# creare-com/pydem

Hardware: AMD Instinct MI355X
Metric: Mcells/s (slope+aspect+UCA+TWI end-to-end) per tile; % HBM roofline (higher is better)
Workload: dtype f64

## Files before the change

pydem_amd/csrc/uca.hip:

```cpp
#include "uca_graph.h"
#include <algorithm>
#include <vector>
#include <math.h>
#include <stdlib.h>
#include <string.h>

#define PI_D 3.141592653589793

namespace {

__global__ __launch_bounds__(256) void k_section_proportion(const double *__restrict__ dir,
                                                            const uint8_t *__restrict__ flats,
                                                            const double *__restrict__ sec_theta, int64_t NN, int n, int m,
                                                            const double *__restrict__ elev,
                                                            int8_t *__restrict__ section, double *__restrict__ prop,
                                                            uint32_t *__restrict__ cinfo)
{
    (void)NN;
    for (int i = blockIdx.y; i < n; i += gridDim.y)
    for (int j = blockIdx.x * blockDim.x + threadIdx.x; j < m; j += gridDim.x * blockDim.x) {
        const int64_t c = (int64_t)i * m + j;
        const double theta = sec_theta[i];
        const double d = dir[c];
        int sec0 = (int)(int8_t)(int)floor(d / PI_D * 2.0);
// ... 431 lines not shown
    uint16_t list[TILE_RING];
    int tail;
    int limit;
};

__device__ __forceinline__ uint16_t &sp_of(TileW &L, int idx) { return reinterpret_cast<uint16_t *>(L.cs)[2 * idx]; }
__device__ __forceinline__ uint32_t sp_state(const TileW &L, int idx) { return (L.cs[idx] >> SP_STATE_SHIFT) & 3u; }

__device__ __forceinline__ uint32_t sp_dec(TileW &L, int idx) { return atomicSub(&L.cs[idx], 1u) & 0xFFFFu; }

__device__ __forceinline__ void tile_wave_sync()
{
    __builtin_amdgcn_fence(__ATOMIC_SEQ_CST, "workgroup");
    __builtin_amdgcn_wave_barrier();
}

__device__ __forceinline__ void tile_lds_sync()
{
    __builtin_amdgcn_fence(__ATOMIC_RELEASE, "workgroup", "local");
    __builtin_amdgcn_wave_barrier();
    __builtin_amdgcn_fence(__ATOMIC_ACQUIRE, "workgroup", "local");
}

constexpr int TILE_PEND = 48;
struct TileNext {
    int32_t *flag;
    int32_t *list, *count;
};

__device__ __forceinline__ const double *in_edge_ptr(const SweepArgs &A, int32_t c, int m, int d)
{
    const int q = d + (d >> 2);
    const int di = (q * 11) >> 5;
    const int32_t u = c + (di - 1) * m + (q - 3 * di - 1);
    return reinterpret_cast<const double *>(A.contrib + u) + (((0x5A >> d) & 1) ? 0 : 1);
}
__device__ __forceinline__ double in_edge(const SweepArgs &A, int32_t c, int m, int d) { return *in_edge_ptr(A, c, m, d); }

struct TileBase {
    const char *cinfo, *area, *contrib, *prop, *todo;
    int32_t org;
};
__device__ __forceinline__ TileBase tile_base(const SweepArgs &A, int i0, int j0)
{
    TileBase B;
    const int64_t org = (int64_t)(i0 - 1) * A.m + (j0 - 1);
// ... 69 lines not shown
            L.fin[HH - 1] = ((br >> 32) << 1) | ((bk >> 2) & 1ull) | (((bk >> 3) & 1ull) << 33);
        }
    }
    constexpr int STG_B = PYDEM_STG_B;
#pragma unroll 1
    for (int kb = 0; kb < NSET; kb += STG_B) {
        uint32_t wst[STG_B];
#pragma unroll
        for (int k = 0; k < STG_B; k++) wst[k] = stage_word(i0 + 2 * (kb + k) + half, j0 + l32);
#pragma unroll
        for (int k = 0; k < STG_B; k++) {
            const int r = 2 * (kb + k);
            const bool f = final_before(wst[k]);
            L.cs[lane + 64 * (kb + k)] = ((wst[k] == 0xFFFFFFFFu ? 0u : (wst[k] & CI_STATIC_MASK)) << 16) | ((f ? 1u : 0u) << SP_STATE_SHIFT);
            const unsigned long long b = __ballot(f);
            if (lane == 0) {
                L.fin[r + 1] = ((b & 0xFFFFFFFFull) << 1) | ((colL >> r) & 1ull) | (((colR >> r) & 1ull) << 33);
                L.fin[r + 2] = ((b >> 32) << 1) | ((colL >> (r + 1)) & 1ull) | (((colR >> (r + 1)) & 1ull) << 33);
            }
        }
    }
}

template <bool LISTED, bool WT = false>
__device__ __forceinline__ void sweep_one_tile(const SweepArgs &A, TileW &L, uint32_t pass, int tiles_x, int tid, int lane,
                                               uint8_t *__restrict__ tile_done, int32_t &n_final, const TileNext &N,
                                               int32_t *pend, int &npend, const int32_t *nbr16)
{
    const int by = tid / tiles_x, bx = tid - by * tiles_x;
    const int i0 = by * TH, j0 = bx * TT, n = A.n, m = A.m;
    const TileBase B = tile_base(A, i0, j0);
    const int half = lane >> 5, l32 = lane & 31;
    auto push_ready = [&](int cell, int consumed) {
        const int slot = atomicAdd(&L.tail, 1);
        if (slot - consumed < TILE_RING) L.list[slot % TILE_RING] = (uint16_t)cell;
        else atomicMin(&L.limit, slot);
    };
#ifdef PYDEM_TILE_PROF
    const bool prof = (A.dbg & 4) != 0 && (int)pass >= (A.dbg >> 8);
#else
    constexpr bool prof = false;
#endif
    long long tk0 = 0, tk1 = 0, tk2 = 0, tk3 = 0;
    int nrounds = 0;
    if (prof) tk0 = wall_clock64();
    if (lane == 0) { L.tail = 0; L.limit = INT32_MAX; }
    const double a0_row = (!WT && lane < TH && i0 + lane < n) ? A.a0[i0 + lane] : 0.0;
    constexpr int NSET = TH * TT / 64;
    tile_stage(A, B, L, pass, i0, j0, lane);
    tile_wave_sync();
    if (prof) tk1 = wall_clock64();
    uint32_t pitmask = 0;
    int32_t n_open = 0;
#pragma unroll 2
    for (int k = 0; k < NSET; k++) {
        const int li = 2 * k + half + 1, idx = lane + 64 * k;
        const uint32_t w = L.cs[idx];
        if (!((w >> SP_STATE_SHIFT) & 3u)) {
            const unsigned long long f0 = L.fin[li - 1], f1 = L.fin[li], f2 = L.fin[li + 1];
            const uint32_t nf = ((uint32_t)(f0 >> l32) & 7u) | (((uint32_t)(f1 >> l32) & 1u) << 3) |
                                (((uint32_t)(f1 >> (l32 + 2)) & 1u) << 4) | (((uint32_t)(f2 >> l32) & 7u) << 5);
            const uint32_t pend = __popc((w >> 16) & 0xFFu & ~nf);
            sp_of(L, idx) = (uint16_t)pend;
            n_open++;
            if (w & (CI_PIT_IN << 16)) pitmask |= 1u << k;
            else if (pend == 0) push_ready(lane + 64 * k, 0);
        }
    }
    if (pitmask) {
        constexpr int PB = 4;
#pragma unroll 1
        for (int kb = 0; kb < NSET; kb += PB) {
            if (!((pitmask >> kb) & ((1u << PB) - 1u))) continue;
            int32_t e0[PB];
#pragma unroll
            for (int k = 0; k < PB; k++) {
                e0[k] = 0;
                if (pitmask & (1u << (kb + k))) {
                    const int cell = lane + 64 * (kb + k);
                    e0[k] = ld_off<int2>(B.area, halo_cell((cell >> 5) + 1, (cell & 31) + 1, m) * 8u).x;
                }
            }
#pragma unroll
            for (int k = 0; k < PB; k++) {
                if (!(pitmask & (1u << (kb + k)))) continue;
                const int cell = lane + 64 * (kb + k);
                const int32_t c = B.org + (int32_t)halo_cell((cell >> 5) + 1, (cell & 31) + 1, m);
                const int idx = cell;
                uint32_t pend = sp_of(L, idx);
// ... 26 lines not shown
    int32_t finalized = 0;
    uint32_t wake = 0;
    int head = 0;
    int mycell = -1, cd = -1;
    double cv = 0.0;
    for (;;) {
        const int tail = L.tail < L.limit ? L.tail : L.limit;
        const bool need = mycell < 0;
        const unsigned long long nb = __ballot(need);
        const int rank = __builtin_amdgcn_mbcnt_hi((uint32_t)(nb >> 32), __builtin_amdgcn_mbcnt_lo((uint32_t)nb, 0u));
        const int avail = tail - head, wanted = __popcll(nb);
        if (need && rank < avail) { mycell = L.list[(head + rank) % TILE_RING]; cd = -1; }
        head += wanted < avail ? wanted : avail;
        if (!__ballot(mycell >= 0)) break;
        nrounds++;
        int next = -1, nd = -1;
        double nv = 0.0;
        if (mycell >= 0) {
            const int cell = mycell;
            const int li = (cell >> 5) + 1, lj = (cell & 31) + 1, idx = cell;
            const int gi = i0 + li - 1, gj = j0 + lj - 1;
            const uint32_t h = halo_cell(li, lj, m);
            const int32_t c = B.org + (int32_t)h;
            const uint32_t cw = L.cs[idx] >> 16;
            double pv = 0.0;
            if (cw & (CI_OUT1 | CI_OUT2)) pv = ld_off<double>(B.prop, h * 8u);
            int2 po = make_int2(0, 0);
            if (cw & (CI_PIT_IN | CI_PIT_OUT)) po = ld_off<int2>(B.area, h * 8u);
            uint32_t mm = cw & 0xFFu;
            double xs[4];
#pragma unroll
            for (int q = 0; q < 4; q++) {
                xs[q] = 0.0;
                if (mm) {
                    const int d = __ffs(mm) - 1; mm &= mm - 1u;
                    if (d == cd) xs[q] = cv; else xs[q] = in_edge_h(B, nbr16, h, d);
                }
            }
            double a;
            bool td;
            if constexpr (WT) {
                a = A.a0[c];
                td = false;
#pragma unroll
                for (int q = 0; q < 4; q++) a += xs[q];
            } else {
                a = L.a0[li - 1];
                td = (gi == 0 || gi == n - 1 || gj == 0 || gj == m - 1) && ld_off<uint8_t>(B.todo, h) != 0;
#pragma unroll
                for (int q = 0; q < 4; q++) { a += fabs(xs[q]); td = td || (xs[q] < 0); }
            }
            while (mm) {
                const int d = __ffs(mm) - 1; mm &= mm - 1u;
                const double x = (d == cd) ? cv : in_edge_h(B, nbr16, h, d);
                if constexpr (WT) a += x;
                else { a += fabs(x); td = td || (x < 0); }
            }
            if (cw & CI_PIT_IN)
                for (int32_t e = po.x; e < A.n_pit && A.pin_dst[e] == c; e++) {
                    const int32_t sc = A.pin_src[e];
                    a += A.area[sc] * A.pin_w[e];
                    if constexpr (!WT) td = td || (A.todo_work[sc] != 0);
                }
            double2 o = make_double2(0.0, 0.0);
            if (cw & CI_OUT1) o.x = a * pv;
            if (cw & CI_OUT2) o.y = a * (1 - pv);
            if (td) { o.x = -o.x; o.y = -o.y; }
            st_off<double>(B.area, h * 8u, a);
#ifndef PYDEM_EXP_NOCONTRIB
            st_off<double2>(B.contrib, h * 16u, o);
#endif
            if (LISTED) st_off<uint32_t>(B.cinfo, h * 4u, ci_with_level(cw, pass));
            if (td) st_off<uint8_t>(B.todo, h, (uint8_t)1);
            sp_of(L, idx) = (uint16_t)(2u << SP_STATE_SHIFT);
            finalized++;
            auto release = [&](int ti, int tj, double share, bool chainable) {
                if (ti >= 1 && ti <= TH && tj >= 1 && tj <= TT) {
                    const int tcell = (ti - 1) * TT + (tj - 1);
                    if (sp_dec(L, tcell) == 1u) {
                        if (chainable && next < 0) {
                            const int q = (li - ti + 1) * 3 + (lj - tj + 1);
                            next = tcell; nd = q - (q > 4 ? 1 : 0); nv = share;
                        } else push_ready(tcell, head);
                    }
                } else if (LISTED) {
                    const int dti = ti < 1 ? -1 : (ti > TH ? 1 : 0), dtj = tj < 1 ? -1 : (tj > TT ? 1 : 0);
                    if (ti >= 1 - TH && ti <= 2 * TH && tj >= 1 - TT && tj <= 2 * TT) wake |= 1u << ((dti + 1) * 3 + dtj + 1);
                    else {
                        const int tt = ((i0 + ti - 1) / TH) * tiles_x + (j0 + tj - 1) / TT;
                        if (atomicExch(&N.flag[tt], (int32_t)pass + 1) != (int32_t)pass + 1) N.list[atomicAdd(N.count, 1)] = tt;
                    }
                }
            };
            const int sct = ci_section(cw);
            if (cw & CI_OUT1) release(li + fe1r(sct), lj + fe1c(sct), o.x, true);
            if (cw & CI_OUT2) release(li + fe2r(sct), lj + fe2c(sct), o.y, true);
            if (cw & CI_PIT_OUT)
                for (int32_t e = po.y; e < A.n_pit && A.pit_src[e] == c; e++) {
                    const int32_t dc = A.pit_dst[e];
                    const int ti = dc / m - i0 + 1, tj = dc % m - j0 + 1;
                    release(ti, tj, 0.0, false);
                }
        }
        mycell = next; cd = nd; cv = nv;
        tile_wave_sync();
    }
    if (prof) tk3 = wall_clock64();
    if (!LISTED)
        for (int k = 0; k < NSET; k++) {
            const int li = 2 * k + half + 1, idx = lane + 64 * k;
            const uint32_t w = L.cs[idx];
            if (((w >> SP_STATE_SHIFT) & 3u) == 2u) A.cinfo[(int64_t)(i0 + li - 1) * m + j0 + l32] = ci_with_level(w >> 16, pass);
        }
    for (int off = 32; off > 0; off >>= 1) { finalized += __shfl_down(finalized, off); n_open += __shfl_down(n_open, off); }
    if (LISTED) {
        for (int off = 32; off > 0; off >>= 1) wake |= __shfl_xor(wake, off);
        bool win = false;
        int tt = 0;
        if (lane < 9 && ((wake >> lane) & 1u)) { tt = tid + (lane / 3 - 1) * tiles_x + (lane % 3 - 1); win = true; }
        if (lane == 9 && L.limit != INT32_MAX) { tt = tid; win = true; }
        if (win) win = atomicExch(&N.flag[tt], (int32_t)pass + 1) != (int32_t)pass + 1;
        const unsigned long long bw = __ballot(win);
        if (win) pend[npend + __popcll(bw & ((1ull << lane) - 1ull))] = tt;
        npend += __popcll(bw);
    }
    if (lane == 0) {
        n_final += finalized;
        if (finalized == n_open) tile_done[tid] = 1;
        A.tile_open[tid] = n_open - finalized;
        if (prof) {
            const long long tk4 = wall_clock64();
            unsigned long long *acc = reinterpret_cast<unsigned long long *>(A.err + (CS_TILE_PROF - CS_QUEUE_ERR));
            atomicAdd(acc + 0, (unsigned long long)(tk1 - tk0)); atomicAdd(acc + 1, (unsigned long long)(tk2 - tk1));
            atomicAdd(acc + 2, (unsigned long long)(tk3 - tk2)); atomicAdd(acc + 3, (unsigned long long)(tk4 - tk3));
            atomicAdd(acc + 4, (unsigned long long)nrounds); atomicAdd(acc + 5, 1ull);
            if (finalized == 0) atomicAdd(acc + 6, 1ull);
        }
    }
    tile_wave_sync();
}

#include "uca_sym.inl"

#ifndef PYDEM_SWEEP_STEAL
#define PYDEM_SWEEP_STEAL 1
#endif
#ifndef PYDEM_FULL_WPB
#define PYDEM_FULL_WPB 4
#endif
constexpr int FWPB = PYDEM_FULL_WPB;
template <bool LISTED, bool WT = false>
__global__ __launch_bounds__(64 * FWPB, 32 / FWPB) void k_sweep_tiles(SweepArgs A, uint32_t pass, int tiles_x, int tiles_total,
                                                     uint8_t *__restrict__ tile_done, int32_t *n_final, TileNext N, int32_t *work8)
{
    __shared__ TileW L[FWPB];
    __shared__ int32_t s_pend[FWPB][TILE_PEND];
    __shared__ int32_t s_nbr16[8];
    fill_nbr16(s_nbr16, A.m);
    __syncthreads();
    const int wave = __builtin_amdgcn_readfirstlane(threadIdx.x >> 6), lane = threadIdx.x & 63;
    int32_t fin = 0;
    int npend = 0;
    auto flush = [&]() {
        tile_wave_sync();
        int32_t base = 0;
// ... 23 lines not shown
            if (tile_done[tid]) continue;
            sweep_one_tile<LISTED, WT>(A, L[wave], pass, tiles_x, tid, lane, tile_done, fin, N, s_pend[wave], npend, s_nbr16);
            if (LISTED && npend > TILE_PEND - 10) flush();
        }
    }
#endif
    if (LISTED && npend) flush();
    if (lane == 0 && fin) atomicAdd(n_final, fin);
}

#ifndef PYDEM_LISTED_OCC
#define PYDEM_LISTED_OCC 6
#endif
#ifndef PYDEM_LISTED_WPB
#define PYDEM_LISTED_WPB 2
#endif
constexpr int LWPB = PYDEM_LISTED_WPB;
template <bool WT = false>
__global__ __launch_bounds__(64 * LWPB, PYDEM_LISTED_OCC) void k_sweep_tiles_listed(SweepArgs A, uint32_t pass, int tiles_x, const int32_t *__restrict__ list_in,
                                                            const int32_t *n_in, uint8_t *__restrict__ tile_done, int32_t *n_final,
                                                            TileNext N, int32_t *clear_count, int32_t *work3, SymArgs Y)
{
    __shared__ TileW L[LWPB];
    __shared__ SymLight SL[LWPB];
    const int wave = threadIdx.x >> 6, lane = threadIdx.x & 63;
    const int32_t nt = *n_in;
#ifdef PYDEM_LISTED_DYNAMIC
    if (blockIdx.x == 0 && threadIdx.x < 8) work3[((pass + 1) % 3) * 8 + threadIdx.x] = 0;
#endif
    if (blockIdx.x == 0 && threadIdx.x == 0) *clear_count = 0;
    __shared__ int32_t s_pend[LWPB][TILE_PEND];
    __shared__ int32_t s_nbr16[8];
    fill_nbr16(s_nbr16, A.m);
    __syncthreads();
    int32_t fin = 0;
    int npend = 0;
    auto flush = [&]() {
        tile_wave_sync();
        int32_t base = 0;
        if (lane == 0) base = atomicAdd(N.count, npend);
        base = __shfl(base, 0);
        if (lane < npend) N.list[base + lane] = s_pend[wave][lane];
        npend = 0;
        tile_wave_sync();
    };
#ifndef PYDEM_LISTED_DYNAMIC
    (void)work3;
    for (int32_t k = __builtin_amdgcn_readfirstlane(blockIdx.x * LWPB + wave); k < nt; k += gridDim.x * LWPB) {
#else
    const int xcd = blockIdx.x & 7;
    const int32_t per = (nt + 7) >> 3;
    int32_t *wk = &work3[(pass % 3) * 8 + xcd];
    for (;;) {
        int32_t k = 0;
        if (lane == 0) k = atomicAdd(wk, 1);
        k = __builtin_amdgcn_readfirstlane(__shfl(k, 0));
        (void)per;
        k = k * 8 + xcd;
        if (k >= nt) break;
#endif
        const int tid = __builtin_amdgcn_readfirstlane(list_in[k]);
        const uint32_t blk = Y.tile_sym ? __builtin_amdgcn_readfirstlane(Y.tile_sym[tid]) : SYM_NONE;
        if (blk != SYM_NONE) sym_light_visit<WT>(A, Y, SL[wave], pass, tiles_x, tid, lane, blk, fin, N, s_pend[wave], npend);
        else sweep_one_tile<true, WT>(A, L[wave], pass, tiles_x, tid, lane, tile_done, fin, N, s_pend[wave], npend, s_nbr16);
        if (npend > TILE_PEND - 10) flush();
    }
    if (npend) flush();
    if (lane == 0 && fin) atomicAdd(n_final, fin);
}

constexpr int DENSE_BAND = 64;
__global__ __launch_bounds__(256) void k_sweep_dense_level(SweepArgs A, uint32_t p, int32_t *n_final)
{
    const int n = A.n, m = A.m;
    int32_t fin = 0;
    const int j = blockIdx.x * blockDim.x + threadIdx.x;
    const int i_end = min(n, (int)(blockIdx.y + 1) * DENSE_BAND);
    if (j < m)
    for (int i = blockIdx.y * DENSE_BAND; i < i_end; i++) {
        const int32_t c = i * m + j;
        const uint32_t w = A.cinfo[c];
        const uint32_t lv = ci_level(w);
        if (lv >= 1 && lv != CI_LEVEL_INF) continue;
        const uint32_t cw = w & CI_STATIC_MASK;
        bool ready = true;
#pragma unroll
        for (int d = 0; d < 8; d++)
// ... 47 lines not shown
constexpr int RCAP = 256;
constexpr uint32_t RS_TAINT = 1u << 19, RS_FIN = 1u << 20;
constexpr int RS_OPEN_SHIFT = 11, RS_FINAL_SHIFT = 21;
constexpr uint32_t RS_CELL = (1u << RS_OPEN_SHIFT) - 1u, RS_CELL_OPEN = (1u << 19) - 1u;

struct TileR {
    TileW W;
    uint16_t map[TH * TT];
    double Kd[RCAP];
    double Pd[RCAP];
    uint32_t sm[RCAP];
};

__device__ __forceinline__ int nb_local(int cell, int d)
{
    const int q = d + (d >> 2);
    const int di = (q * 11) >> 5;
    return cell + (di - 1) * TT + (q - 3 * di - 1);
}

template <bool WT = false>
__device__ __forceinline__ void sweep_tile_resident(const SweepArgs &A, TileR &R, uint32_t pass, int tiles_x, int tid, int lane,
                                                    uint8_t *__restrict__ tile_done, int32_t &n_final, const TileNext &N,
                                                    int32_t *pend, int &npend)
{
    TileW &L = R.W;
    const int by = tid / tiles_x, bx = tid - by * tiles_x;
    const int i0 = by * TH, j0 = bx * TT, n = A.n, m = A.m;
    const int half = lane >> 5, l32 = lane & 31;
    constexpr int NSET = TH * TT / 64;
    if (lane == 0) L.tail = 0;
    const double a0_row = (!WT && lane < TH && i0 + lane < n) ? A.a0[i0 + lane] : 0.0;
    tile_stage(A, tile_base(A, i0, j0), L, pass, i0, j0, lane);
    tile_wave_sync();
    uint32_t pitmask = 0;
    int nslot = 0;
#pragma unroll 2
    for (int k = 0; k < NSET; k++) {
        const int li = 2 * k + half + 1, idx = lane + 64 * k;
        const uint32_t w = L.cs[idx];
        const bool open = !((w >> SP_STATE_SHIFT) & 3u);
        const unsigned long long bo = __ballot(open);
        if (open) {
            const unsigned long long f0 = L.fin[li - 1], f1 = L.fin[li], f2 = L.fin[li + 1];
            const uint32_t nf = ((uint32_t)(f0 >> l32) & 7u) | (((uint32_t)(f1 >> l32) & 1u) << 3) |
                                (((uint32_t)(f1 >> (l32 + 2)) & 1u) << 4) | (((uint32_t)(f2 >> l32) & 7u) << 5);
            const uint32_t im = (w >> 16) & 0xFFu;
            const uint32_t cnt = __popc(im & ~nf);
            sp_of(L, idx) = (uint16_t)cnt;
            const int s = nslot + __popcll(bo & ((1ull << lane) - 1ull));
            R.map[idx] = (uint16_t)s;
            R.sm[s] = (uint32_t)idx | ((im & ~nf) << RS_OPEN_SHIFT) | ((im & nf) << RS_FINAL_SHIFT);
            if (w & (CI_PIT_IN << 16)) pitmask |= 1u << k;
            else if (cnt == 0) L.list[atomicAdd(&L.tail, 1)] = (uint16_t)s;
        }
        nslot += __popcll(bo);
    }
    if (pitmask) {
#pragma unroll 1
        for (int k = 0; k < NSET; k++) {
            if (!(pitmask & (1u << k))) continue;
            const int cell = lane + 64 * k;
            const int32_t c = (i0 + (cell >> 5)) * m + j0 + (cell & 31);
            uint32_t cnt = sp_of(L, cell);
            for (int32_t e = pit_stash(A, c).x; e < A.n_pit && A.pin_dst[e] == c; e++) {
                const int32_t sc = A.pin_src[e];
                const int si = sc / m - i0, sj = sc % m - j0;
                if (si >= 0 && si < TH && sj >= 0 && sj < TT) cnt += sp_state(L, si * TT + sj) ? 0u : 1u;
                else { const uint32_t lv = ci_level(A.cinfo[sc]); if (!(lv >= 1 && lv < pass)) cnt |= SP_BLOCKED; }
            }
            sp_of(L, cell) = (uint16_t)cnt;
            if (cnt == 0) L.list[atomicAdd(&L.tail, 1)] = R.map[cell];
        }
    }
    tile_wave_sync();
    if (lane < TH) L.a0[lane] = a0_row;
    tile_wave_sync();
    for (int s = lane; s < nslot; s += 64) {
        uint32_t smv = R.sm[s];
        const int cell = smv & RS_CELL;
        const int gi = i0 + (cell >> 5), gj = j0 + (cell & 31);
        const int32_t c = gi * m + gj;
        const uint32_t cw = L.cs[cell] >> 16;
        double pv = 0.0;
        if (cw & (CI_OUT1 | CI_OUT2)) pv = A.prop[c];
        bool td = !WT && (gi == 0 || gi == n - 1 || gj == 0 || gj == m - 1) && A.todo_work[c] != 0;
        uint32_t mm = (smv >> RS_FINAL_SHIFT) & 0xFFu;
        double xs[4];
#pragma unroll
        for (int q = 0; q < 4; q++) {
            xs[q] = 0.0;
            if (mm) { const int d = __ffs(mm) - 1; mm &= mm - 1u; xs[q] = in_edge(A, c, m, d); }
        }
        double K;
        if constexpr (WT) {
// ... 1 lines not shown
#pragma unroll
            for (int q = 0; q < 4; q++) K += xs[q];
            while (mm) { const int d = __ffs(mm) - 1; mm &= mm - 1u; K += in_edge(A, c, m, d); }
        } else {
            K = L.a0[cell >> 5];
#pragma unroll
            for (int q = 0; q < 4; q++) { K += fabs(xs[q]); td = td || (xs[q] < 0); }
            while (mm) { const int d = __ffs(mm) - 1; mm &= mm - 1u; const double x = in_edge(A, c, m, d); K += fabs(x); td = td || (x < 0); }
        }
        R.Kd[s] = K; R.Pd[s] = pv;
        R.sm[s] = (smv & RS_CELL_OPEN) | (td ? RS_TAINT : 0u);
    }
    tile_lds_sync();
    uint32_t wake = 0;
    int head = 0;
    for (;;) {
        const int tail = L.tail;
        if (head >= tail) break;
        const int idx = head + lane;
        if (idx < tail) {
            const int s = L.list[idx];
            const uint32_t smv = R.sm[s];
            const int cell = smv & RS_CELL, li = cell >> 5, lj = cell & 31;
            const uint32_t cw = L.cs[cell] >> 16;
            double a = R.Kd[s];
            bool td = (smv & RS_TAINT) != 0u;
            uint32_t mm = (smv >> RS_OPEN_SHIFT) & 0xFFu;
            while (mm) {
                const int d = __ffs(mm) - 1; mm &= mm - 1u;
                const int ss = R.map[nb_local(cell, d)];
                const double as = R.Kd[ss], ps = R.Pd[ss];
                a += ((0x5A >> d) & 1) ? as * ps : as * (1 - ps);
                td = td || (R.sm[ss] & RS_TAINT);
            }
            const int32_t c = (i0 + li) * m + j0 + lj;
            int2 po = make_int2(0, 0);
            if (cw & (CI_PIT_IN | CI_PIT_OUT)) po = pit_stash(A, c);
            if (cw & CI_PIT_IN)
                for (int32_t e = po.x; e < A.n_pit && A.pin_dst[e] == c; e++) {
                    const int32_t sc = A.pin_src[e];
                    const int si = sc / m - i0, sj = sc % m - j0;
                    bool here = false;
                    if (si >= 0 && si < TH && sj >= 0 && sj < TT) here = sp_state(L, si * TT + sj) == 2u;
                    if (here) { const int ss = R.map[si * TT + sj]; a += R.Kd[ss] * A.pin_w[e]; td = td || (R.sm[ss] & RS_TAINT); }
                    else { a += A.area[sc] * A.pin_w[e]; if constexpr (!WT) td = td || (A.todo_work[sc] != 0); }
                }
            R.Kd[s] = a;
            R.sm[s] = (smv & RS_CELL) | (td ? RS_TAINT : 0u) | RS_FIN;
            sp_of(L, cell) = (uint16_t)(2u << SP_STATE_SHIFT);
            auto release = [&](int ti, int tj) {
                if (ti >= 0 && ti < TH && tj >= 0 && tj < TT) {
                    const int tcell = ti * TT + tj;
                    if (sp_dec(L, tcell) == 1u) L.list[atomicAdd(&L.tail, 1)] = R.map[tcell];
                } else {
                    const int dti = ti < 0 ? -1 : (ti >= TH ? 1 : 0), dtj = tj < 0 ? -1 : (tj >= TT ? 1 : 0);
                    if (ti >= -TH && ti < 2 * TH && tj >= -TT && tj < 2 * TT) wake |= 1u << ((dti + 1) * 3 + dtj + 1);
                    else {
                        const int tt = ((i0 + ti) / TH) * tiles_x + (j0 + tj) / TT;
                        if (atomicExch(&N.flag[tt], (int32_t)pass + 1) != (int32_t)pass + 1) N.list[atomicAdd(N.count, 1)] = tt;
                    }
                }
            };
            const int sct = ci_section(cw);
            if (cw & CI_OUT1) release(li + fe1r(sct), lj + fe1c(sct));
            if (cw & CI_OUT2) release(li + fe2r(sct), lj + fe2c(sct));
            if (cw & CI_PIT_OUT)
                for (int32_t e = po.y; e < A.n_pit && A.pit_src[e] == c; e++) {
                    const int32_t dc = A.pit_dst[e];
                    release(dc / m - i0, dc % m - j0);
                }
        }
        head = tail < head + 64 ? tail : head + 64;
        tile_lds_sync();
    }
    int nfin = 0;
    for (int s = lane; s < nslot; s += 64) {
        const uint32_t smv = R.sm[s];
        if (!(smv & RS_FIN)) continue;
        const int cell = smv & RS_CELL;
        const int32_t c = (i0 + (cell >> 5)) * m + j0 + (cell & 31);
        const uint32_t cw = L.cs[cell] >> 16;
        const double a = R.Kd[s], pv = R.Pd[s];
        double2 o = make_double2(0.0, 0.0);
        if (cw & CI_OUT1) o.x = a * pv;
        if (cw & CI_OUT2) o.y = a * (1 - pv);
        if (smv & RS_TAINT) { o.x = -o.x; o.y = -o.y; A.todo_work[c] = 1; }
        A.area[c] = a;
        A.contrib[c] = o;
        A.cinfo[c] = ci_with_level(cw, pass);
        nfin++;
    }
    for (int off = 32; off > 0; off >>= 1) { nfin += __shfl_down(nfin, off); wake |= __shfl_xor(wake, off); }
    bool win = false;
    int tt = 0;
    if (lane < 9 && ((wake >> lane) & 1u)) { tt = tid + (lane / 3 - 1) * tiles_x + (lane % 3 - 1); win = true; }
    if (win) win = atomicExch(&N.flag[tt], (int32_t)pass + 1) != (int32_t)pass + 1;
    const unsigned long long bw = __ballot(win);
    if (win) pend[npend + __popcll(bw & ((1ull << lane) - 1ull))] = tt;
    npend += __popcll(bw);
    if (lane == 0) {
        n_final += nfin;
        A.tile_open[tid] = nslot - nfin;
        if (nfin == nslot) tile_done[tid] = 1;
    }
    tile_wave_sync();
}

template <bool WT = false>
__global__ __launch_bounds__(64) void k_sweep_tiles_resident(SweepArgs A, uint32_t pass, int tiles_x, const int32_t *__restrict__ list_in,
                                                             const int32_t *n_in, uint8_t *__restrict__ tile_done, int32_t *n_final,
                                                             TileNext N, int32_t *clear_count, SymArgs Y)
{
    __shared__ TileR R;
    __shared__ SymLight SL;
    __shared__ int32_t s_pend[TILE_PEND];
    __shared__ int32_t s_nbr16[8];
    fill_nbr16(s_nbr16, A.m);
    __syncthreads();
    const int lane = threadIdx.x;
    const int32_t nt = *n_in;
    if (blockIdx.x == 0 && lane == 0) *clear_count = 0;
    int32_t fin = 0;
    int npend = 0;
    auto flush = [&]() {
        tile_wave_sync();
        int32_t base = 0;
        if (lane == 0) base = atomicAdd(N.count, npend);
        base = __shfl(base, 0);
        if (lane < npend) N.list[base + lane] = s_pend[lane];
        npend = 0;
        tile_wave_sync();
    };
    for (int32_t k = blockIdx.x; k < nt; k += gridDim.x) {
        const int tid = __builtin_amdgcn_readfirstlane(list_in[k]);
        const uint32_t blk = Y.tile_sym ? __builtin_amdgcn_readfirstlane(Y.tile_sym[tid]) : SYM_NONE;
        if (blk != SYM_NONE) sym_light_visit<WT>(A, Y, SL, pass, tiles_x, tid, lane, blk, fin, N, s_pend, npend);
        else if (__builtin_amdgcn_readfirstlane(A.tile_open[tid]) <= RCAP)
            sweep_tile_resident<WT>(A, R, pass, tiles_x, tid, lane, tile_done, fin, N, s_pend, npend);
        else
            sweep_one_tile<true, WT>(A, R.W, pass, tiles_x, tid, lane, tile_done, fin, N, s_pend, npend, s_nbr16);
        if (npend > TILE_PEND - 10) flush();
    }
    if (npend) flush();
    if (lane == 0 && fin) atomicAdd(n_final, fin);
}

constexpr uint32_t FC_COUNT = 0xFu, FC_BLOCKED = 1u << 8, FC_DONE = 1u << 9, FC_TODO = 1u << 10;

struct TileFirst {
    double2 slot[TT * TT];
    uint32_t cs[TT * TT];
    double a0[TT];
};

__device__ __forceinline__ void lds_sync()
{
    __builtin_amdgcn_fence(__ATOMIC_RELEASE, "workgroup", "local");
    __builtin_amdgcn_s_barrier();
    __builtin_amdgcn_fence(__ATOMIC_ACQUIRE, "workgroup", "local");
}

__global__ __launch_bounds__(256) void k_sweep_first(SweepArgs A, int tiles_x, int tiles_total, uint8_t *__restrict__ tile_done,
                                                     int32_t *n_final)
// ... 960 lines not shown
```

pydem_amd/csrc/uca_graph.h:

```cpp
#pragma once
#include "internal.h"
#include <stdlib.h>

namespace {

constexpr uint32_t CI_OUT1 = 1u << 8, CI_OUT2 = 1u << 9, CI_PIT_OUT = 1u << 10, CI_PIT_IN = 1u << 11;
constexpr int CI_SEC_SHIFT = 12, CI_LEVEL_SHIFT = 15;
constexpr uint32_t CI_LEVEL_INF = 0x1FFFFu, CI_STATIC_MASK = 0x7FFFu;
__device__ __forceinline__ uint32_t ci_level(uint32_t w) { return w >> CI_LEVEL_SHIFT; }
__device__ __forceinline__ int ci_section(uint32_t w) { return (int)((w >> CI_SEC_SHIFT) & 7u); }
__device__ __forceinline__ uint32_t ci_with_level(uint32_t w, uint32_t lv) { return (w & CI_STATIC_MASK) | (lv << CI_LEVEL_SHIFT); }

__device__ __constant__ const int NB_DI[8] = {-1, -1, -1, 0, 0, 1, 1, 1};
__device__ __constant__ const int NB_DJ[8] = {-1, 0, 1, -1, 1, -1, 0, 1};
__device__ __constant__ const int NB_S0[8] = {6, 5, 4, 0, 3, 0, 1, 2};
__device__ __constant__ const int NB_S1[8] = {7, 6, 5, 7, 4, 1, 2, 3};

__device__ __forceinline__ bool keep_edge(double w, double z_to, double z_from)
{
    return !isnan(w) && (w > 1e-8) && (z_to <= z_from);
}

struct SweepArgs {
    uint32_t *cinfo;
    const double *prop, *a0;
    double *area;
    double2 *contrib;
    uint8_t *todo_work;
    int n, m;
    const int32_t *pit_src, *pit_dst;
    const int32_t *pin_dst, *pin_src; const double *pin_w;
    int64_t n_pit;
    int dbg;
    int32_t qcap;
    int32_t *err;
    int32_t *tile_open;
};

struct QE { int32_t c; uint32_t cw; };

enum CounterSlot : int {
    CS_FRONTIER = 0,
    CS_PROCESSED = 3,
    CS_SOURCES = 4,
    CS_ROUNDS = 5,
    CS_EDGE_REACHED = 6,
    CS_EDGE_CLEARED = 7,
    CS_EDGE_SEEDS = 8,
    CS_CASCADE_STATE = 12,
    CS_SWEEP_STATE = 14,
    CS_QUEUE_ERR = 15,
    CS_WINDOW = 16,
    CS_H_CB_TOTALS = 16,
    CS_WORK = 16, CS_WORK_WORDS = 24,
    CS_TILE_PROF = 32, CS_TILE_PROF_WORDS = 24,
    CS_EINC_PROF = 40,
// ... 9 lines not shown
static_assert(CS_FRONTIER + 3 <= CS_PROCESSED && CS_ROUNDS == CS_PROCESSED + 2, "kernels reach the round count through the processed-cells pointer");
static_assert(CS_ROUNDS < CS_EDGE_REACHED && CS_EDGE_SEEDS < CS_CASCADE_STATE && CS_CASCADE_STATE < CS_SWEEP_STATE && CS_SWEEP_STATE < CS_QUEUE_ERR,
              "the scalars of a cascade are live together");
static_assert(CS_QUEUE_ERR < CS_WINDOW && CS_WINDOW <= CS_WORK, "one copy of the window shows the host every scalar of a cascade, and no scratch");
static_assert(CS_WORK + CS_WORK_WORDS <= CS_EINC_PROF, "zeroing the per-tile scratch leaves the fix-up's words alone");
static_assert(CS_TILE_PROF + CS_TILE_PROF_WORDS <= CS_TILE_LIST, "the visit profile ends before the tile lists");
static_assert(CS_EINC_PROF + 8 <= CS_ND_COUNT && CS_ND_COUNT + 2 <= CS_ND_NEXT && CS_ND_NEXT < CS_NAN_SEEDS && CS_NAN_SEEDS < CS_COND_EDGES
              && CS_COND_EDGES < CS_TILE_LIST, "the fix-up's words are live together and stay clear of the sweep's");
static_assert(CS_TILE_LIST + 4 <= CS_RESEED && CS_RESEED + 3 <= CS_END && CS_FLAT_SAVE + 2 <= CS_END, "the sweep's lists and replay words are live together");

inline int grid_for(int64_t work, int cap) { const int64_t g = cdiv(work, 256); return (int)(g < cap ? (g > 0 ? g : 1) : cap); }
}

static void fill_sweep_args(pydem_tile *t, SweepArgs &A)
{
    A.cinfo = t->cinfo; A.prop = t->prop; A.a0 = t->row_area; A.area = t->uca;
    A.contrib = (double2 *)t->contrib; A.todo_work = t->todo_work; A.n = (int)t->n; A.m = (int)t->m;
    A.pit_src = t->pits.src; A.pit_dst = t->pits.dst; A.n_pit = t->pits.n_edges;
    A.pin_dst = t->pits.in_dst; A.pin_src = t->pits.in_src; A.pin_w = t->pits.in_w;
    A.qcap = (int32_t)(t->NN / 2 < INT32_MAX ? t->NN / 2 : INT32_MAX);
    A.err = t->counters + CS_QUEUE_ERR;
    A.tile_open = nullptr;
    { const char *e = getenv("PYDEM_TILE_DEBUG"); A.dbg = e ? atoi(e) : 0; }
}
```

Before: 5750.

## Stage pit edge lists in LDS during listed tile sweeps

```diff
diff --git a/pydem_amd/csrc/uca.hip b/pydem_amd/csrc/uca.hip
--- a/pydem_amd/csrc/uca.hip
+++ b/pydem_amd/csrc/uca.hip
@@ -477,6 +477,69 @@
     __builtin_amdgcn_fence(__ATOMIC_ACQUIRE, "workgroup", "local");
 }
 
+constexpr int PS_CAP = 120;
+constexpr int PS_CELLS = 64;
+constexpr int PS_END = 0xFF;
+constexpr uint32_t CW_STAGED = 1u << 15;
+constexpr int SP_HEAD_SHIFT = 6;
+constexpr uint32_t SP_STAGED_COUNT = (1u << SP_HEAD_SHIFT) - 1u, SP_STAGED_READY = (3u << SP_STATE_SHIFT) | SP_BLOCKED | SP_STAGED_COUNT;
+constexpr int32_t PS_NBR = TH * TT, PS_FAR = 1 << 30;
+static_assert((CI_STATIC_MASK & CW_STAGED) == 0 && PS_CAP <= PS_END && ((PS_CAP - 1) << SP_HEAD_SHIFT) < (int)SP_BLOCKED, "pit staging layout");
+struct PitStage {
+    int32_t a[PS_CAP];
+    int32_t e[PS_CAP];
+    uint8_t nxt[PS_CAP];
+    uint16_t cells[PS_CELLS];
+    int n, nc;
+};
+
+__device__ __forceinline__ bool sp_dec_ready(TileW &L, int idx)
+{
+    const uint32_t old = atomicSub(&L.cs[idx], 1u);
+    return (old & ((old >> 31) ? SP_STAGED_READY : 0xFFFFu)) == 1u;
+}
+
+__device__ __forceinline__ bool ps_append(PitStage &P, int &first, int &prev, int32_t av, int32_t ev)
+{
+    const int q = atomicAdd(&P.n, 1);
+    if (q >= PS_CAP) return false;
+    P.a[q] = av; P.e[q] = ev; P.nxt[q] = (uint8_t)PS_END;
+    if (prev < 0) first = q; else P.nxt[prev] = (uint8_t)q;
+    prev = q;
+    return true;
+}
+__device__ __forceinline__ int32_t ps_out_code(int32_t dc, int m, int i0, int j0, int tiles_x)
+{
+    const int gi = dc / m, gj = dc - gi * m;
+    const int ti = gi - i0, tj = gj - j0;
+    if (ti >= 0 && ti < TH && tj >= 0 && tj < TT) return ti * TT + tj;
+    if (ti >= -TH && ti < 2 * TH && tj >= -TT && tj < 2 * TT)
+        return PS_NBR + ((ti < 0 ? 0 : (ti >= TH ? 2 : 1)) * 3 + (tj < 0 ? 0 : (tj >= TT ? 2 : 1)));
+    return PS_FAR | ((gi / TH) * tiles_x + gj / TT);
+}
+__device__ __forceinline__ bool ps_stage_out(const SweepArgs &A, PitStage &P, int32_t c, int32_t e0, int i0, int j0, int tiles_x,
+                                             int &first, int &prev)
+{
+    const int m = A.m;
+    bool fits = true;
+    for (int32_t e = e0; fits; e += 2) {
+        const int64_t ia = e < A.n_pit ? e : A.n_pit - 1, ib = e + 1 < A.n_pit ? e + 1 : A.n_pit - 1;
+        const int32_t sa = A.pit_src[ia], sb = A.pit_src[ib], da = A.pit_dst[ia], db = A.pit_dst[ib];
+        const bool va = e < A.n_pit && sa == c, vb = va && e + 1 < A.n_pit && sb == c;
+        if (va) fits = fits && ps_append(P, first, prev, ps_out_code(da, m, i0, j0, tiles_x), -1);
+        if (vb) fits = fits && ps_append(P, first, prev, ps_out_code(db, m, i0, j0, tiles_x), -1);
+        if (!vb) break;
+    }
+    return fits;
+}
+__device__ __forceinline__ void ps_flag(TileW &L, int idx, int first)
+{
+    const uint32_t spv = sp_of(L, idx);
+    if (first < 0 || (spv & (SP_BLOCKED - 1u)) > SP_STAGED_COUNT) return;
+    sp_of(L, idx) = (uint16_t)(spv | ((uint32_t)first << SP_HEAD_SHIFT));
+    reinterpret_cast<uint16_t *>(L.cs)[2 * idx + 1] |= (uint16_t)CW_STAGED;
+}
+
 constexpr int TILE_PEND = 48;
 struct TileNext {
     int32_t *flag;
@@ -592,11 +655,13 @@
     }
 }
 
-template <bool LISTED, bool WT = false>
+template <bool LISTED, bool WT = false, bool STAGE = false>
 __device__ __forceinline__ void sweep_one_tile(const SweepArgs &A, TileW &L, uint32_t pass, int tiles_x, int tid, int lane,
                                                uint8_t *__restrict__ tile_done, int32_t &n_final, const TileNext &N,
-                                               int32_t *pend, int &npend, const int32_t *nbr16)
-{
+                                               int32_t *pend, int &npend, const int32_t *nbr16, PitStage *P = nullptr)
+{
+    static_assert(!STAGE || LISTED, "pit staging: listed visits only");
+    const bool staging = STAGE && A.pitstage != 0;
     const int by = tid / tiles_x, bx = tid - by * tiles_x;
     const int i0 = by * TH, j0 = bx * TT, n = A.n, m = A.m;
     const TileBase B = tile_base(A, i0, j0);
@@ -614,7 +679,7 @@
     long long tk0 = 0, tk1 = 0, tk2 = 0, tk3 = 0;
     int nrounds = 0;
     if (prof) tk0 = wall_clock64();
-    if (lane == 0) { L.tail = 0; L.limit = INT32_MAX; }
+    if (lane == 0) { L.tail = 0; L.limit = INT32_MAX; if (STAGE) { P->n = 0; P->nc = 0; } }
     const double a0_row = (!WT && lane < TH && i0 + lane < n) ? A.a0[i0 + lane] : 0.0;
     constexpr int NSET = TH * TT / 64;
     tile_stage(A, B, L, pass, i0, j0, lane);
@@ -633,8 +698,72 @@
             const uint32_t pend = __popc((w >> 16) & 0xFFu & ~nf);
             sp_of(L, idx) = (uint16_t)pend;
             n_open++;
-            if (w & (CI_PIT_IN << 16)) pitmask |= 1u << k;
+            bool listed = false;
+            if constexpr (STAGE) {
+                if (staging && (w & ((CI_PIT_IN | CI_PIT_OUT) << 16))) {
+                    const int q = atomicAdd(&P->nc, 1);
+                    if (q < PS_CELLS) { P->cells[q] = (uint16_t)idx; listed = true; }
+                }
+            }
+            if (w & (CI_PIT_IN << 16)) { if (!listed) pitmask |= 1u << k; }
             else if (pend == 0) push_ready(lane + 64 * k, 0);
+        }
+    }
+    if constexpr (STAGE) {
+        if (staging) {
+            tile_lds_sync();
+            const int nc = P->nc < PS_CELLS ? P->nc : PS_CELLS;
+            const int64_t last = A.n_pit - 1;
+            auto at = [&](int32_t e) -> int64_t { return e < A.n_pit ? (int64_t)e : last; };
+#pragma unroll 1
+            for (int base = 0; base < nc; base += 64) {
+                if (base + lane >= nc) continue;
+                const int cell = P->cells[base + lane];
+                const uint32_t cwh = L.cs[cell] >> 16;
+                const uint32_t hc = halo_cell((cell >> 5) + 1, (cell & 31) + 1, m);
+                const int32_t c = B.org + (int32_t)hc;
+                const int2 e0 = ld_off<int2>(B.area, hc * 8u);
+                const bool isin = (cwh & CI_PIT_IN) != 0u, isout = (cwh & CI_PIT_OUT) != 0u;
+                const int32_t ei = isin ? e0.x : 0, eo = isout ? e0.y : 0;
+                int32_t da = A.pin_dst[at(ei)], db = A.pin_dst[at(ei + 1)], sa = A.pin_src[at(ei)], sb = A.pin_src[at(ei + 1)];
+                int32_t osa = A.pit_src[at(eo)], osb = A.pit_src[at(eo + 1)], oda = A.pit_dst[at(eo)], odb = A.pit_dst[at(eo + 1)];
+                int first = -1, prev = -1;
+                bool fits = true;
+                if (isin) {
+                    uint32_t pend = sp_of(L, cell);
+                    for (int32_t e = ei;;) {
+                        const bool va = e < A.n_pit && da == c, vb = va && e + 1 < A.n_pit && db == c;
+                        auto blocked = [&](int32_t sc) -> uint32_t {
+                            const int si = sc / m - i0, sj = sc % m - j0;
+                            if (si >= 0 && si < TH && sj >= 0 && sj < TT)
+                                return sp_state(L, si * TT + sj) ? 0u : 1u;
+                            const uint32_t lv = ci_level(A.cinfo[sc]);
+                            return (lv >= 1 && lv < pass) ? 0u : SP_BLOCKED;
+                        };
+                        uint32_t ba = 0, bb = 0;
+                        if (va) ba = blocked(sa);
+                        if (vb) bb = blocked(sb);
+                        pend = (pend + (ba & 1u) + (bb & 1u)) | ((ba | bb) & SP_BLOCKED);
+                        if (va) fits = fits && ps_append(*P, first, prev, sa, e);
+                        if (vb) fits = fits && ps_append(*P, first, prev, sb, e + 1);
+                        if (!vb) break;
+                        e += 2;
+                        da = A.pin_dst[at(e)]; db = A.pin_dst[at(e + 1)]; sa = A.pin_src[at(e)]; sb = A.pin_src[at(e + 1)];
+                    }
+                    sp_of(L, cell) = (uint16_t)pend;
+                    if (pend == 0) push_ready(cell, 0);
+                }
+                if (isout)
+                    for (int32_t e = eo; fits;) {
+                        const bool va = e < A.n_pit && osa == c, vb = va && e + 1 < A.n_pit && osb == c;
+                        if (va) fits = fits && ps_append(*P, first, prev, ps_out_code(oda, m, i0, j0, tiles_x), -1);
+                        if (vb) fits = fits && ps_append(*P, first, prev, ps_out_code(odb, m, i0, j0, tiles_x), -1);
+                        if (!vb) break;
+                        e += 2;
+                        osa = A.pit_src[at(e)]; osb = A.pit_src[at(e + 1)]; oda = A.pit_dst[at(e)]; odb = A.pit_dst[at(e + 1)];
+                    }
+                if (fits) ps_flag(L, cell, first);
+            }
         }
     }
     if (pitmask) {
@@ -707,11 +836,26 @@
             const int gi = i0 + li - 1, gj = j0 + lj - 1;
             const uint32_t h = halo_cell(li, lj, m);
             const int32_t c = B.org + (int32_t)h;
-            const uint32_t cw = L.cs[idx] >> 16;
+            const uint32_t w0 = L.cs[idx], cw = w0 >> 16;
             double pv = 0.0;
             if (cw & (CI_OUT1 | CI_OUT2)) pv = ld_off<double>(B.prop, h * 8u);
             int2 po = make_int2(0, 0);
-            if (cw & (CI_PIT_IN | CI_PIT_OUT)) po = ld_off<int2>(B.area, h * 8u);
+            const bool stg = STAGE && (cw & CW_STAGED);
+            if ((cw & (CI_PIT_IN | CI_PIT_OUT)) && !stg) po = ld_off<int2>(B.area, h * 8u);
+            int sk = PS_END;
+            double pa0 = 0.0, pw0 = 0.0;
+            uint8_t pt0 = 0;
+            if constexpr (STAGE) {
+                if (stg) {
+                    sk = (int)((w0 >> SP_HEAD_SHIFT) & 0x7Fu);
+                    if (cw & CI_PIT_IN) {
+                        const int32_t sc = P->a[sk], e = P->e[sk];
+                        sk = P->nxt[sk];
+                        pa0 = A.area[sc]; pw0 = A.pin_w[e];
+                        if constexpr (!WT) pt0 = A.todo_work[sc];
+                    }
+                }
+            }
             uint32_t mm = cw & 0xFFu;
             double xs[4];
 #pragma unroll
@@ -741,12 +885,23 @@
                 if constexpr (WT) a += x;
                 else { a += fabs(x); td = td || (x < 0); }
             }
-            if (cw & CI_PIT_IN)
-                for (int32_t e = po.x; e < A.n_pit && A.pin_dst[e] == c; e++) {
-                    const int32_t sc = A.pin_src[e];
-                    a += A.area[sc] * A.pin_w[e];
-                    if constexpr (!WT) td = td || (A.todo_work[sc] != 0);
-                }
+            if (cw & CI_PIT_IN) {
+                if (stg) {
+                    a += pa0 * pw0;
+                    if constexpr (!WT) td = td || (pt0 != 0);
+                    while (sk != PS_END && P->e[sk] >= 0) {
+                        const int32_t sc = P->a[sk], e = P->e[sk];
+                        sk = P->nxt[sk];
+                        a += A.area[sc] * A.pin_w[e];
+                        if constexpr (!WT) td = td || (A.todo_work[sc] != 0);
+                    }
+                } else
+                    for (int32_t e = po.x; e < A.n_pit && A.pin_dst[e] == c; e++) {
+                        const int32_t sc = A.pin_src[e];
+                        a += A.area[sc] * A.pin_w[e];
+                        if constexpr (!WT) td = td || (A.todo_work[sc] != 0);
+                    }
+            }
             double2 o = make_double2(0.0, 0.0);
             if (cw & CI_OUT1) o.x = a * pv;
             if (cw & CI_OUT2) o.y = a * (1 - pv);
@@ -762,7 +917,7 @@
             auto release = [&](int ti, int tj, double share, bool chainable) {
                 if (ti >= 1 && ti <= TH && tj >= 1 && tj <= TT) {
                     const int tcell = (ti - 1) * TT + (tj - 1);
-                    if (sp_dec(L, tcell) == 1u) {
+                    if (STAGE ? sp_dec_ready(L, tcell) : sp_dec(L, tcell) == 1u) {
                         if (chainable && next < 0) {
                             const int q = (li - ti + 1) * 3 + (lj - tj + 1);
                             next = tcell; nd = q - (q > 4 ? 1 : 0); nv = share;
@@ -780,12 +935,25 @@
             const int sct = ci_section(cw);
             if (cw & CI_OUT1) release(li + fe1r(sct), lj + fe1c(sct), o.x, true);
             if (cw & CI_OUT2) release(li + fe2r(sct), lj + fe2c(sct), o.y, true);
-            if (cw & CI_PIT_OUT)
-                for (int32_t e = po.y; e < A.n_pit && A.pit_src[e] == c; e++) {
-                    const int32_t dc = A.pit_dst[e];
-                    const int ti = dc / m - i0 + 1, tj = dc % m - j0 + 1;
-                    release(ti, tj, 0.0, false);
-                }
+            if (cw & CI_PIT_OUT) {
+                if (stg) {
+                    while (sk != PS_END) {
+                        const int32_t code = P->a[sk];
+                        sk = P->nxt[sk];
+                        if (code < PS_NBR) release((code >> 5) + 1, (code & 31) + 1, 0.0, false);
+                        else if (code < PS_FAR) wake |= 1u << (code - PS_NBR);
+                        else {
+                            const int tt = code & (PS_FAR - 1);
+                            if (atomicExch(&N.flag[tt], (int32_t)pass + 1) != (int32_t)pass + 1) N.list[atomicAdd(N.count, 1)] = tt;
+                        }
+                    }
+                } else
+                    for (int32_t e = po.y; e < A.n_pit && A.pit_src[e] == c; e++) {
+                        const int32_t dc = A.pit_dst[e];
+                        const int ti = dc / m - i0 + 1, tj = dc % m - j0 + 1;
+                        release(ti, tj, 0.0, false);
+                    }
+            }
         }
         mycell = next; cd = nd; cv = nv;
         tile_wave_sync();
@@ -826,6 +994,8 @@
 }
 
 #include "uca_sym.inl"
+
+union VisitScratch { SymLight sl; PitStage ps; };
 
 #ifndef PYDEM_SWEEP_STEAL
 #define PYDEM_SWEEP_STEAL 1
@@ -895,7 +1065,7 @@
                                                             TileNext N, int32_t *clear_count, int32_t *work3, SymArgs Y)
 {
     __shared__ TileW L[LWPB];
-    __shared__ SymLight SL[LWPB];
+    __shared__ VisitScratch VS[LWPB];
     const int wave = threadIdx.x >> 6, lane = threadIdx.x & 63;
     const int32_t nt = *n_in;
 #ifdef PYDEM_LISTED_DYNAMIC
@@ -934,8 +1104,8 @@
 #endif
         const int tid = __builtin_amdgcn_readfirstlane(list_in[k]);
         const uint32_t blk = Y.tile_sym ? __builtin_amdgcn_readfirstlane(Y.tile_sym[tid]) : SYM_NONE;
-        if (blk != SYM_NONE) sym_light_visit<WT>(A, Y, SL[wave], pass, tiles_x, tid, lane, blk, fin, N, s_pend[wave], npend);
-        else sweep_one_tile<true, WT>(A, L[wave], pass, tiles_x, tid, lane, tile_done, fin, N, s_pend[wave], npend, s_nbr16);
+        if (blk != SYM_NONE) sym_light_visit<WT>(A, Y, VS[wave].sl, pass, tiles_x, tid, lane, blk, fin, N, s_pend[wave], npend);
+        else sweep_one_tile<true, WT, true>(A, L[wave], pass, tiles_x, tid, lane, tile_done, fin, N, s_pend[wave], npend, s_nbr16, &VS[wave].ps);
         if (npend > TILE_PEND - 10) flush();
     }
     if (npend) flush();
@@ -1029,18 +1199,19 @@
 template <bool WT = false>
 __device__ __forceinline__ void sweep_tile_resident(const SweepArgs &A, TileR &R, uint32_t pass, int tiles_x, int tid, int lane,
                                                     uint8_t *__restrict__ tile_done, int32_t &n_final, const TileNext &N,
-                                                    int32_t *pend, int &npend)
+                                                    int32_t *pend, int &npend, PitStage &P)
 {
     TileW &L = R.W;
+    const bool staging = A.pitstage != 0;
     const int by = tid / tiles_x, bx = tid - by * tiles_x;
     const int i0 = by * TH, j0 = bx * TT, n = A.n, m = A.m;
     const int half = lane >> 5, l32 = lane & 31;
     constexpr int NSET = TH * TT / 64;
-    if (lane == 0) L.tail = 0;
+    if (lane == 0) { L.tail = 0; P.n = 0; }
     const double a0_row = (!WT && lane < TH && i0 + lane < n) ? A.a0[i0 + lane] : 0.0;
     tile_stage(A, tile_base(A, i0, j0), L, pass, i0, j0, lane);
     tile_wave_sync();
-    uint32_t pitmask = 0;
+    uint32_t pitmask = 0, pomask = 0;
     int nslot = 0;
 #pragma unroll 2
     for (int k = 0; k < NSET; k++) {
@@ -1060,24 +1231,34 @@
             R.sm[s] = (uint32_t)idx | ((im & ~nf) << RS_OPEN_SHIFT) | ((im & nf) << RS_FINAL_SHIFT);
             if (w & (CI_PIT_IN << 16)) pitmask |= 1u << k;
             else if (cnt == 0) L.list[atomicAdd(&L.tail, 1)] = (uint16_t)s;
+            if (staging && (w & (CI_PIT_OUT << 16))) pomask |= 1u << k;
         }
         nslot += __popcll(bo);
     }
-    if (pitmask) {
+    if (pitmask | pomask) {
 #pragma unroll 1
         for (int k = 0; k < NSET; k++) {
-            if (!(pitmask & (1u << k))) continue;
+            if (!((pitmask | pomask) & (1u << k))) continue;
             const int cell = lane + 64 * k;
             const int32_t c = (i0 + (cell >> 5)) * m + j0 + (cell & 31);
-            uint32_t cnt = sp_of(L, cell);
-            for (int32_t e = pit_stash(A, c).x; e < A.n_pit && A.pin_dst[e] == c; e++) {
-                const int32_t sc = A.pin_src[e];
-                const int si = sc / m - i0, sj = sc % m - j0;
-                if (si >= 0 && si < TH && sj >= 0 && sj < TT) cnt += sp_state(L, si * TT + sj) ? 0u : 1u;
-                else { const uint32_t lv = ci_level(A.cinfo[sc]); if (!(lv >= 1 && lv < pass)) cnt |= SP_BLOCKED; }
-            }
-            sp_of(L, cell) = (uint16_t)cnt;
-            if (cnt == 0) L.list[atomicAdd(&L.tail, 1)] = R.map[cell];
+            const int2 e0 = pit_stash(A, c);
+            int first = -1, prev = -1;
+            bool fits = true;
+            if (pitmask & (1u << k)) {
+                uint32_t cnt = sp_of(L, cell);
+                for (int32_t e = e0.x; e < A.n_pit && A.pin_dst[e] == c; e++) {
+                    const int32_t sc = A.pin_src[e];
+                    const int si = sc / m - i0, sj = sc % m - j0;
+                    const bool inside = si >= 0 && si < TH && sj >= 0 && sj < TT;
+                    if (inside) cnt += sp_state(L, si * TT + sj) ? 0u : 1u;
+                    else { const uint32_t lv = ci_level(A.cinfo[sc]); if (!(lv >= 1 && lv < pass)) cnt |= SP_BLOCKED; }
+                    if (staging) fits = fits && ps_append(P, first, prev, inside ? -1 - (si * TT + sj) : sc, e);
+                }
+                sp_of(L, cell) = (uint16_t)cnt;
+                if (cnt == 0) L.list[atomicAdd(&L.tail, 1)] = R.map[cell];
+            }
+            if (fits && (pomask & (1u << k))) fits = ps_stage_out(A, P, c, e0.y, i0, j0, tiles_x, first, prev);
+            if (staging && fits) ps_flag(L, cell, first);
         }
     }
     tile_wave_sync();
@@ -1125,7 +1306,9 @@
             const int s = L.list[idx];
             const uint32_t smv = R.sm[s];
             const int cell = smv & RS_CELL, li = cell >> 5, lj = cell & 31;
-            const uint32_t cw = L.cs[cell] >> 16;
+            const uint32_t w0 = L.cs[cell], cw = w0 >> 16;
+            const bool stg = (cw & CW_STAGED) != 0u;
+            int sk = stg ? (int)((w0 >> SP_HEAD_SHIFT) & 0x7Fu) : PS_END;
             double a = R.Kd[s];
             bool td = (smv & RS_TAINT) != 0u;
             uint32_t mm = (smv >> RS_OPEN_SHIFT) & 0xFFu;
@@ -1138,23 +1321,37 @@
             }
             const int32_t c = (i0 + li) * m + j0 + lj;
             int2 po = make_int2(0, 0);
-            if (cw & (CI_PIT_IN | CI_PIT_OUT)) po = pit_stash(A, c);
-            if (cw & CI_PIT_IN)
-                for (int32_t e = po.x; e < A.n_pit && A.pin_dst[e] == c; e++) {
-                    const int32_t sc = A.pin_src[e];
-                    const int si = sc / m - i0, sj = sc % m - j0;
-                    bool here = false;
-                    if (si >= 0 && si < TH && sj >= 0 && sj < TT) here = sp_state(L, si * TT + sj) == 2u;
-                    if (here) { const int ss = R.map[si * TT + sj]; a += R.Kd[ss] * A.pin_w[e]; td = td || (R.sm[ss] & RS_TAINT); }
-                    else { a += A.area[sc] * A.pin_w[e]; if constexpr (!WT) td = td || (A.todo_work[sc] != 0); }
-                }
+            if ((cw & (CI_PIT_IN | CI_PIT_OUT)) && !stg) po = pit_stash(A, c);
+            if (cw & CI_PIT_IN) {
+                if (stg) {
+                    while (sk != PS_END && P.e[sk] >= 0) {
+                        const int32_t av = P.a[sk], e = P.e[sk];
+                        sk = P.nxt[sk];
+                        const int lc = -1 - av;
+                        if (av < 0 && sp_state(L, lc) == 2u) {
+                            const int ss = R.map[lc]; a += R.Kd[ss] * A.pin_w[e]; td = td || (R.sm[ss] & RS_TAINT);
+                        } else {
+                            const int32_t sc = av < 0 ? (i0 + (lc >> 5)) * m + j0 + (lc & 31) : av;
+                            a += A.area[sc] * A.pin_w[e]; if constexpr (!WT) td = td || (A.todo_work[sc] != 0);
+                        }
+                    }
+                } else
+                    for (int32_t e = po.x; e < A.n_pit && A.pin_dst[e] == c; e++) {
+                        const int32_t sc = A.pin_src[e];
+                        const int si = sc / m - i0, sj = sc % m - j0;
+                        bool here = false;
+                        if (si >= 0 && si < TH && sj >= 0 && sj < TT) here = sp_state(L, si * TT + sj) == 2u;
+                        if (here) { const int ss = R.map[si * TT + sj]; a += R.Kd[ss] * A.pin_w[e]; td = td || (R.sm[ss] & RS_TAINT); }
+                        else { a += A.area[sc] * A.pin_w[e]; if constexpr (!WT) td = td || (A.todo_work[sc] != 0); }
+                    }
+            }
             R.Kd[s] = a;
             R.sm[s] = (smv & RS_CELL) | (td ? RS_TAINT : 0u) | RS_FIN;
             sp_of(L, cell) = (uint16_t)(2u << SP_STATE_SHIFT);
             auto release = [&](int ti, int tj) {
                 if (ti >= 0 && ti < TH && tj >= 0 && tj < TT) {
                     const int tcell = ti * TT + tj;
-                    if (sp_dec(L, tcell) == 1u) L.list[atomicAdd(&L.tail, 1)] = R.map[tcell];
+                    if (sp_dec_ready(L, tcell)) L.list[atomicAdd(&L.tail, 1)] = R.map[tcell];
                 } else {
                     const int dti = ti < 0 ? -1 : (ti >= TH ? 1 : 0), dtj = tj < 0 ? -1 : (tj >= TT ? 1 : 0);
                     if (ti >= -TH && ti < 2 * TH && tj >= -TT && tj < 2 * TT) wake |= 1u << ((dti + 1) * 3 + dtj + 1);
@@ -1167,11 +1364,24 @@
             const int sct = ci_section(cw);
             if (cw & CI_OUT1) release(li + fe1r(sct), lj + fe1c(sct));
             if (cw & CI_OUT2) release(li + fe2r(sct), lj + fe2c(sct));
-            if (cw & CI_PIT_OUT)
-                for (int32_t e = po.y; e < A.n_pit && A.pit_src[e] == c; e++) {
-                    const int32_t dc = A.pit_dst[e];
-                    release(dc / m - i0, dc % m - j0);
-                }
+            if (cw & CI_PIT_OUT) {
+                if (stg) {
+                    while (sk != PS_END) {
+                        const int32_t code = P.a[sk];
+                        sk = P.nxt[sk];
+                        if (code < PS_NBR) release(code >> 5, code & 31);
+                        else if (code < PS_FAR) wake |= 1u << (code - PS_NBR);
+                        else {
+                            const int tt = code & (PS_FAR - 1);
+                            if (atomicExch(&N.flag[tt], (int32_t)pass + 1) != (int32_t)pass + 1) N.list[atomicAdd(N.count, 1)] = tt;
+                        }
+                    }
+                } else
+                    for (int32_t e = po.y; e < A.n_pit && A.pit_src[e] == c; e++) {
+                        const int32_t dc = A.pit_dst[e];
+                        release(dc / m - i0, dc % m - j0);
+                    }
+            }
         }
         head = tail < head + 64 ? tail : head + 64;
         tile_lds_sync();
@@ -1215,7 +1425,7 @@
                                                              TileNext N, int32_t *clear_count, SymArgs Y)
 {
     __shared__ TileR R;
-    __shared__ SymLight SL;
+    __shared__ VisitScratch VS;
     __shared__ int32_t s_pend[TILE_PEND];
     __shared__ int32_t s_nbr16[8];
     fill_nbr16(s_nbr16, A.m);
@@ -1237,11 +1447,11 @@
     for (int32_t k = blockIdx.x; k < nt; k += gridDim.x) {
         const int tid = __builtin_amdgcn_readfirstlane(list_in[k]);
         const uint32_t blk = Y.tile_sym ? __builtin_amdgcn_readfirstlane(Y.tile_sym[tid]) : SYM_NONE;
-        if (blk != SYM_NONE) sym_light_visit<WT>(A, Y, SL, pass, tiles_x, tid, lane, blk, fin, N, s_pend, npend);
+        if (blk != SYM_NONE) sym_light_visit<WT>(A, Y, VS.sl, pass, tiles_x, tid, lane, blk, fin, N, s_pend, npend);
         else if (__builtin_amdgcn_readfirstlane(A.tile_open[tid]) <= RCAP)
-            sweep_tile_resident<WT>(A, R, pass, tiles_x, tid, lane, tile_done, fin, N, s_pend, npend);
+            sweep_tile_resident<WT>(A, R, pass, tiles_x, tid, lane, tile_done, fin, N, s_pend, npend, VS.ps);
         else
-            sweep_one_tile<true, WT>(A, R.W, pass, tiles_x, tid, lane, tile_done, fin, N, s_pend, npend, s_nbr16);
+            sweep_one_tile<true, WT, true>(A, R.W, pass, tiles_x, tid, lane, tile_done, fin, N, s_pend, npend, s_nbr16, &VS.ps);
         if (npend > TILE_PEND - 10) flush();
     }
     if (npend) flush();
diff --git a/pydem_amd/csrc/uca_graph.h b/pydem_amd/csrc/uca_graph.h
--- a/pydem_amd/csrc/uca_graph.h
+++ b/pydem_amd/csrc/uca_graph.h
@@ -32,6 +32,7 @@
     const int32_t *pin_dst, *pin_src; const double *pin_w;
     int64_t n_pit;
     int dbg;
+    int pitstage;
     int32_t qcap;
     int32_t *err;
     int32_t *tile_open;
@@ -87,4 +88,7 @@
     A.err = t->counters + CS_QUEUE_ERR;
     A.tile_open = nullptr;
     { const char *e = getenv("PYDEM_TILE_DEBUG"); A.dbg = e ? atoi(e) : 0; }
+    static int pitstage = -1;
+    if (pitstage < 0) { const char *e = getenv("PYDEM_SWEEP_PITSTAGE"); pitstage = (e && atoi(e) == 0) ? 0 : 1; }
+    A.pitstage = pitstage;
 }
```

After: 5849 (median of 6 runs). No clear change (+1.7%).
